# danieleschmidt/Graph-Hypernetwork-Forge

Hardware: AMD Instinct MI355X
Metric: edges/s (HyperGNN forward) (higher is better)
Workload: dtype f32; 1 GPU; synthetic uniform KG 1M nodes / 10M edges / 64 rel, hidden 128, L=3 (BASELINE config 3); nodes=1000000, edges=10000000, relations=64, hidden_dim=128, layers=3, text_dim=64, plan=cached (warm), launch=one C-ABI call per kernel, parallelism=single GPU

## Files before the change

graph-hypernetwork-forge_amd/csrc/message_bx.hip:

```cpp
#include "common.h"

#include <type_traits>

namespace ghf {

typedef float f32x4 __attribute__((ext_vector_type(4)));
typedef int i32x4 __attribute__((ext_vector_type(4)));
typedef int i32x2 __attribute__((ext_vector_type(2)));
typedef float f32x2 __attribute__((ext_vector_type(2)));
typedef _Float16 f16x8 __attribute__((ext_vector_type(8)));
typedef _Float16 f16x4 __attribute__((ext_vector_type(4)));
typedef __attribute__((address_space(3))) void* lptr_t;

template <class T>
__device__ __forceinline__ const T* bx_at(const void* base, uint32_t byte_off) {
    return (const T*)((const char*)base + byte_off);
}

__device__ __forceinline__ int lds_ld_b32(unsigned addr) {
    int v;
    asm volatile("ds_read_b32 %0, %1\n\ts_waitcnt lgkmcnt(0)" : "=&v"(v) : "v"(addr) : "memory");
    return v;
}
__device__ __forceinline__ void lds_ld_b32_x2(unsigned a0, unsigned a1, int& v0, int& v1) {
    asm volatile("ds_read_b32 %0, %2\n\tds_read_b32 %1, %3\n\ts_waitcnt lgkmcnt(0)" : "=&v"(v0), "=&v"(v1) : "v"(a0), "v"(a1) : "memory");
}
__device__ __forceinline__ void lds_ld_b32_x6(const unsigned (&a)[6], int (&v)[6]) {
    asm volatile("ds_read_b32 %0, %6\n\tds_read_b32 %1, %7\n\tds_read_b32 %2, %8\n\tds_read_b32 %3, %9\n\tds_read_b32 %4, %10\n\t"
                 "ds_read_b32 %5, %11\n\ts_waitcnt lgkmcnt(0)"
                 : "=&v"(v[0]), "=&v"(v[1]), "=&v"(v[2]), "=&v"(v[3]), "=&v"(v[4]), "=&v"(v[5])
                 : "v"(a[0]), "v"(a[1]), "v"(a[2]), "v"(a[3]), "v"(a[4]), "v"(a[5]) : "memory");
}
__device__ __forceinline__ void lds_ld_b32_x10(const unsigned (&a)[10], int (&v)[10]) {
    asm volatile("ds_read_b32 %0, %10\n\tds_read_b32 %1, %11\n\tds_read_b32 %2, %12\n\tds_read_b32 %3, %13\n\tds_read_b32 %4, %14\n\t"
                 "ds_read_b32 %5, %15\n\tds_read_b32 %6, %16\n\tds_read_b32 %7, %17\n\tds_read_b32 %8, %18\n\tds_read_b32 %9, %19\n\t"
                 "s_waitcnt lgkmcnt(0)"
                 : "=&v"(v[0]), "=&v"(v[1]), "=&v"(v[2]), "=&v"(v[3]), "=&v"(v[4]), "=&v"(v[5]), "=&v"(v[6]), "=&v"(v[7]), "=&v"(v[8]), "=&v"(v[9])
                 : "v"(a[0]), "v"(a[1]), "v"(a[2]), "v"(a[3]), "v"(a[4]), "v"(a[5]), "v"(a[6]), "v"(a[7]), "v"(a[8]), "v"(a[9]) : "memory");
}
__device__ __forceinline__ void lds_ld_b64_x2(unsigned a0, unsigned a1, f32x2& v0, f32x2& v1) {
    asm volatile("ds_read_b64 %0, %2\n\tds_read_b64 %1, %3\n\ts_waitcnt lgkmcnt(0)" : "=&v"(v0), "=&v"(v1) : "v"(a0), "v"(a1) : "memory");
}
__device__ __forceinline__ void lds_st_b32(unsigned addr, int v) { asm volatile("ds_write_b32 %0, %1" ::"v"(addr), "v"(v) : "memory"); }
__device__ __forceinline__ void lds_st_b64(unsigned addr, f32x2 v) { asm volatile("ds_write_b64 %0, %1" ::"v"(addr), "v"(v) : "memory"); }
__device__ __forceinline__ void lds_st_b128(unsigned addr, f32x4 v) { asm volatile("ds_write_b128 %0, %1" ::"v"(addr), "v"(v) : "memory"); }
#define BX_LGKM0() asm volatile("s_waitcnt lgkmcnt(0)" ::: "memory")
__device__ __forceinline__ int opaque_lane(int lane) {
    int z;
    asm volatile("v_mov_b32 %0, 0" : "=v"(z));
    return lane + z;
}

__device__ __forceinline__ int fresh_lane() {
    int z;
    asm volatile("v_mov_b32 %0, 0" : "=v"(z));
    return (int)__builtin_amdgcn_mbcnt_hi(~0u, __builtin_amdgcn_mbcnt_lo(~0u, (unsigned)z));
}

template <class T> __device__ __forceinline__ T bx_tail_ld(const T* p) { return __builtin_nontemporal_load(p); }
template <class T> __device__ __forceinline__ void bx_tail_st(T* p, T v) { __builtin_nontemporal_store(v, p); }
#define BX_IDX_WAIT "s_nop 3\n\t"
constexpr int BX_AD = 2, BX_TGB = 3;
constexpr int BX_FSPLIT = 8;

template <int D> struct BxCfg;
template <> struct BxCfg<128> {
    static constexpr int NPW = 96, CR = 76;
    static constexpr int BN = 4 * NPW;
    static constexpr int MTC = (CR + 15) / 16;
    static constexpr bool DEFER = true;
    static constexpr size_t LDS = (size_t)4 * 2 * CR * 256 + 4 * (4 * 16 * MTC + 4) * 4 + 1024 + 512 + 64;
};
template <> struct BxCfg<64> {
    static constexpr int NPW = 48, CR = 64;
    static constexpr int BN = 4 * NPW;
    static constexpr int MTC = (CR + 15) / 16;
    static constexpr bool DEFER = false;
    static constexpr size_t LDS = (size_t)4 * 2 * CR * 128 + 4 * (4 * 16 * MTC + 4) * 4 + 1024 + 512 + 64;
};

typedef float f32x32 __attribute__((ext_vector_type(32)));
typedef float f32x16 __attribute__((ext_vector_type(16)));
#define BX_PIN_128(s) "+{v[64:95]}"(s[0]), "+{v[96:127]}"(s[1]), "+{v[128:159]}"(s[2]), "+{v[160:191]}"(s[3]), "+{v[192:223]}"(s[4]), "+{v[224:255]}"(s[5])
#define BX_PIN_64(s) "+{v[64:79]}"(s[0]), "+{v[80:95]}"(s[1]), "+{v[96:111]}"(s[2])

struct BxChunk { int r; int e0; int rows; };

template <int GB_, int NV_> struct BxTailSt {
    static constexpr int GB = GB_, NV = NV_;
    f32x4 x[GB_][NV_];
    int deg[GB_];
    float gm[4 * NV_], bt[4 * NV_];
};
constexpr int BX_TCG = 8;

template <int D, int SKIP>
__global__ __launch_bounds__(512, D == 64 ? 4 : 2) void message_bx_kernel(
    const float* __restrict__ h, const void* __restrict__ h_split, int64_t N, const uint32_t* __restrict__ sorted_key,
    const int32_t* __restrict__ sorted_src, const int32_t* __restrict__ chunk_tab,
    const int32_t* __restrict__ item_tab, int64_t item0, float* __restrict__ partial,
    const int32_t* __restrict__ indeg, int R,
    const void* __restrict__ Wsplit, const float* __restrict__ bias,
    const float* __restrict__ gamma, const float* __restrict__ beta, float eps,
    int64_t row0, int64_t row_end, float* __restrict__ h_out, void* __restrict__ h_split_out, int no_tail,
    int32_t* __restrict__ range_flag, float* __restrict__ agg_out) {
    using C = BxCfg<D>;
    constexpr bool SWAP1 = SKIP == 1;
    constexpr int skip = SWAP1 ? 2 : SKIP;
    constexpr int P0_IDS = SWAP1 ? 3 : 2;
    constexpr int P0_HALF = SWAP1 ? 1 : 0;
    constexpr int BN = C::BN, MTC = C::MTC, CR = C::CR, NPW = C::NPW;
    constexpr bool DEFER = C::DEFER;
    constexpr int NWV = 8, TW = 4;
    constexpr int KS = D / 32;
    constexpr int NKS = 2 * KS;
    constexpr int NT = D / 16;
    constexpr int NTW = NT / TW;
    constexpr int NPL = 2;
    constexpr int ROWB = D * 2;
    constexpr int PLANE = CR * ROWB;
    constexpr int TILE = NPL * PLANE;
    constexpr int HROW = NPL * D * 2;
    constexpr int CRP = 16 * MTC;
    constexpr int MSTR = 4 * CRP + 4;
    constexpr int PL = D / 64;
    constexpr int TUP = D == 128 ? 32 : 16;
    constexpr int NSV = NPW * PL / TUP;
    constexpr int RPP = 1024 / ROWB;
    constexpr int LPR = 64 / RPP;
    constexpr int RBN = CR / RPP;
    constexpr int CPL = D / 16;
    constexpr int RBW = (RBN + TW - 1) / TW;
    constexpr int RPH = (CR + TW - 1) / TW;
    static_assert((NTW == 2 || NTW == 1) && CR % RPP == 0 && RPH <= 64 && NPW * TW == BN && (NPW * PL) % TUP == 0 && NPW * PL <= 192 &&
                      NPW % 2 == 0 && (BN / 2) % 4 == 0 && CR <= 128 && NSV <= 6 && (D == 128 || D == 64), "bad config");
    auto akey = [](int row) -> int { return D == 128 ? (row & 15) : ((row >> 1) & 7); };
    constexpr unsigned META_OFF = 4 * TILE,
                       DUMMY_OFF = META_OFF + 4 * MSTR * 4, ZERO_OFF = DUMMY_OFF + 1024,
                       FLAG_OFF = ZERO_OFF + 512;
    auto tile_of = [](int j) -> unsigned { return (unsigned)(j & 3) * (unsigned)TILE; };

    extern __shared__ __attribute__((aligned(16))) char smem[];
    const unsigned lds0 = (unsigned)(size_t)(lptr_t)smem;

    const int tid = threadIdx.x, lane = tid & 63;
    const int w = __builtin_amdgcn_readfirstlane(tid >> 6);
    const bool helper = w >= TW;
    const int tw = w & 3;
    const int q = lane >> 4, c16 = lane & 15;
    const i32x4 item = *(const i32x4*)(item_tab + 4 * (size_t)(item0 + blockIdx.x));
    const int64_t blk = __builtin_amdgcn_readfirstlane(item[0]);
    const int slot = __builtin_amdgcn_readfirstlane(item[3]);
    const int64_t node0 = blk * BN;
    const int nrows = (int)((row_end - node0) < BN ? (row_end - node0) : BN);
    const uint32_t seg0 = (uint32_t)(blk * R);
    const int c_begin = __builtin_amdgcn_readfirstlane(item[1]);
    const int c_end = __builtin_amdgcn_readfirstlane(item[2]);
    const int nchunks = c_end - c_begin;
    int vzero;
    asm volatile("v_mov_b32 %0, 0" : "=v"(vzero));

    auto load_desc = [&](int k) -> i32x2 {
        const int c = c_begin + (k < nchunks ? k : 0) + vzero;
        return *bx_at<i32x2>(chunk_tab, (uint32_t)c * 8u);
    };
    auto decode = [&](i32x2 d) -> BxChunk {
        const int w0 = __builtin_amdgcn_readfirstlane(d[0]), w1 = __builtin_amdgcn_readfirstlane(d[1]);
        return BxChunk{w1 >> 8, w0, w1 & 127};
    };
    auto meta_off = [&](int j) -> unsigned { return META_OFF + (unsigned)(j & 3) * (MSTR * 4); };
    const uint32_t hsc_off = (uint32_t)((uint64_t)N * HROW);

    constexpr int HN = BN / 2, HPW = NPW / 2;
    auto tail_half = [&](int half, auto gb_c) __attribute__((always_inline)) {
        const float* acc_lds = (const float*)smem;
        constexpr int CS = 64;
        const int sub = lane >> 4, c0 = 4 * (lane & 15);
        constexpr int NV = CPL / 4;
        auto node_of = [&](int v) -> int { return (v / HPW) * NPW + half * HPW + (v % HPW); };
        auto row_sum = [&](float v) -> float {
            v += dpp_take<0xB1, 0xF>(v);
            v += dpp_take<0x4E, 0xF>(v);
            v += dpp_take<0x141, 0xF>(v);
            v += dpp_take<0x140, 0xF>(v);
            return v;
        };
        auto row_max = [&](float v) -> float {
            v = fmaxf(v, dpp_take<0xB1, 0xF>(v));
            v = fmaxf(v, dpp_take<0x4E, 0xF>(v));
            v = fmaxf(v, dpp_take<0x141, 0xF>(v));
            v = fmaxf(v, dpp_take<0x140, 0xF>(v));
            return v;
        };
        constexpr int NG = HN / 4;
        if (slot >= 0) {
            float* __restrict__ ps = partial + (size_t)slot * BN * D;
            for (int g = w; g < NG; g += NWV) {
                const int v = 4 * g + sub;
                float* __restrict__ o = ps + (size_t)node_of(v) * D + c0;
#pragma unroll
                for (int i = 0; i < NV; ++i) *(f32x4*)(o + CS * i) = *(const f32x4*)(acc_lds + v * D + c0 + CS * i);
            }
            return;
        }
        float gm[CPL], bt[CPL];
#pragma unroll
        for (int c = 0; c < CPL; ++c) {
            gm[c] = no_tail ? 1.f : gamma[c0 + CS * (c >> 2) + (c & 3)];
            bt[c] = no_tail ? 0.f : beta[c0 + CS * (c >> 2) + (c & 3)];
        }
        constexpr int GB = decltype(gb_c)::value;
        for (int g0 = w; g0 < NG; g0 += NWV * GB) {
            f32x4 x[GB][NV];
            float inv[GB];
            int deg[GB];
#pragma unroll
            for (int gb = 0; gb < GB; ++gb) {
                const int g = g0 + gb * NWV;
                const int nl = node_of(4 * (g < NG ? g : NG - 1) + sub);
                const int64_t node = node0 + (nl < nrows ? nl : nrows - 1);
                deg[gb] = indeg[node];
                const float* __restrict__ hp = h + (size_t)node * D + c0;
#pragma unroll
                for (int i = 0; i < NV; ++i)
                    x[gb][i] = (no_tail && !(no_tail & GHF_FLAG_ADD_H)) ? (f32x4){0.f, 0.f, 0.f, 0.f} : bx_tail_ld((const f32x4*)(hp + CS * i));
            }
            __builtin_amdgcn_sched_barrier(0);
#pragma unroll
            for (int gb = 0; gb < GB; ++gb) inv[gb] = (no_tail & GHF_FLAG_RAW_SUM) ? 1.0f : 1.0f / (float)(deg[gb] > 1 ? deg[gb] : 1);
#pragma unroll
            for (int gb = 0; gb < GB; ++gb) {
                const int g = g0 + gb * NWV;
                const int v = 4 * (g < NG ? g : NG - 1) + sub;
                const int nl = node_of(v);
                const bool live = g < NG && nl < nrows;
                f32x4 a[NV];
#pragma unroll
                for (int i = 0; i < NV; ++i) a[i] = *(const f32x4*)(acc_lds + v * D + c0 + CS * i);
                if (agg_out && live) {
                    float* __restrict__ o = agg_out + (size_t)(node0 + nl) * D + c0;
#pragma unroll
                    for (int i = 0; i < NV; ++i) bx_tail_st((f32x4*)(o + CS * i), a[i] * inv[gb]);
                }
                float y[CPL];
                float s = 0.f;
#pragma unroll
                for (int c = 0; c < CPL; ++c) {
                    const float av = a[c >> 2][c & 3] * inv[gb];
                    y[c] = no_tail ? av + x[gb][c >> 2][c & 3] : fmaxf(av + x[gb][c >> 2][c & 3], 0.f);
                    s += y[c];
                }
                if (!no_tail) {
                    const float mean = row_sum(s) * (1.0f / D);
                    float var = 0.f;
#pragma unroll
                    for (int c = 0; c < CPL; ++c) { const float t = y[c] - mean; var += t * t; }
                    const float rstd = 1.0f / sqrtf(row_sum(var) * (1.0f / D) + eps);
#pragma unroll
                    for (int c = 0; c < CPL; ++c) y[c] = (y[c] - mean) * rstd * gm[c] + bt[c];
                }
                float up = 1.f;
                if (h_split_out) {
                    float mx = 0.f;
#pragma unroll
                    for (int c = 0; c < CPL; ++c) mx = fmaxf(mx, fabsf(y[c]));
                    const int sh = split2h_shift(row_max(mx));
                    up = pow2f(sh);
                    if ((lane & 15) == 0 && live) *(float*)((char*)h_split_out + (size_t)hsc_off + (size_t)(node0 + nl) * 4) = pow2f(-sh);
                }
                if (live) {
                    float* __restrict__ o = h_out + (size_t)(node0 + nl) * D + c0;
#pragma unroll
                    for (int i = 0; i < NV; ++i) bx_tail_st((f32x4*)(o + CS * i), (f32x4){y[4 * i], y[4 * i + 1], y[4 * i + 2], y[4 * i + 3]});
                    if (h_split_out) {
                        _Float16* __restrict__ sp = (_Float16*)h_split_out + (size_t)(node0 + nl) * (NPL * D) + c0;
                        _Float16 hi[CPL], lo[CPL];
#pragma unroll
                        for (int c = 0; c < CPL; ++c) split2h(y[c] * up, hi[c], lo[c]);
                        if constexpr (CPL == 8 && CS == 4) {
                            *(f16x8*)sp = (f16x8){hi[0], hi[1], hi[2], hi[3], hi[4], hi[5], hi[6], hi[7]};
                            *(f16x8*)(sp + D) = (f16x8){lo[0], lo[1], lo[2], lo[3], lo[4], lo[5], lo[6], lo[7]};
                        } else if constexpr (CPL == 8) {
#pragma unroll
                            for (int i = 0; i < 2; ++i) {
                                bx_tail_st((f16x4*)(sp + CS * i), (f16x4){hi[4 * i], hi[4 * i + 1], hi[4 * i + 2], hi[4 * i + 3]});
                                bx_tail_st((f16x4*)(sp + D + CS * i), (f16x4){lo[4 * i], lo[4 * i + 1], lo[4 * i + 2], lo[4 * i + 3]});
                            }
                        } else {
                            bx_tail_st((f16x4*)sp, (f16x4){hi[0], hi[1], hi[2], hi[3]});
                            bx_tail_st((f16x4*)(sp + D), (f16x4){lo[0], lo[1], lo[2], lo[3]});
                        }
                    }
                }
                if (h_split_out) {
                    int tiny = 0, nz = 0;
#pragma unroll
                    for (int c = 0; c < CPL; ++c) { tiny += range_tiny(y[c] * up); nz += y[c] != 0.f; }
                    if (__ballot(tiny != 0)) {
                        tiny = (int)row_sum((float)tiny);
                        nz = (int)row_sum((float)nz);
                        if ((lane & 15) == 0 && live) range_raise(range_flag, GHF_RANGE_ROWS, tiny, nz);
                    }
                }
            }
        }
    };

    auto tail_issue = [&](int half, auto& st, int gfirst, auto gend_c) __attribute__((always_inline)) {
        using St = typename std::remove_reference<decltype(st)>::type;
        constexpr int GB = St::GB, NV = St::NV, CS = 64;
        static_assert(NV * 4 == CPL && 4 * GB <= decltype(gend_c)::value, "one batch holds all of the wave's groups");
        if (slot >= 0) return;
        const int tl = fresh_lane(), sub = tl >> 4, c0 = 4 * (tl & 15);
        const bool no_x = no_tail && !(no_tail & GHF_FLAG_ADD_H);
        const __amdgpu_buffer_rsrc_t rsG = __builtin_amdgcn_make_buffer_rsrc((void*)gamma, 0, no_tail ? 0 : D * 4, 0x00020000);
        const __amdgpu_buffer_rsrc_t rsB = __builtin_amdgcn_make_buffer_rsrc((void*)beta, 0, no_tail ? 0 : D * 4, 0x00020000);
        const __amdgpu_buffer_rsrc_t rsX = __builtin_amdgcn_make_buffer_rsrc(
            (void*)h, 0, no_x ? 0 : (int)(uint32_t)((uint64_t)N * D * 4), 0x00020000);
#pragma unroll
        for (int c = 0; c < CPL; ++c) {
            st.gm[c] = __builtin_bit_cast(float, __builtin_amdgcn_raw_buffer_load_b32(rsG, (c0 + CS * (c >> 2) + (c & 3)) * 4, 0, 0));
            st.bt[c] = __builtin_bit_cast(float, __builtin_amdgcn_raw_buffer_load_b32(rsB, (c0 + CS * (c >> 2) + (c & 3)) * 4, 0, 0));
        }
#pragma unroll
        for (int gb = 0; gb < GB; ++gb) {
            const int v = 4 * (gfirst + 4 * gb) + sub;
            const int nl = (v / HPW) * NPW + half * HPW + (v % HPW);
            const int64_t node = node0 + (nl < nrows ? nl : nrows - 1);
            st.deg[gb] = indeg[node];
#pragma unroll
            for (int i = 0; i < NV; ++i)
                st.x[gb][i] = __builtin_bit_cast(f32x4, __builtin_amdgcn_raw_buffer_load_b128(
                    rsX, (int)(((uint32_t)node * D + c0 + CS * i) * 4u), 0, 2 ));
        }
        __builtin_amdgcn_sched_barrier(0);
    };
    auto tail_rows = [&](int half, auto& st, int gfirst, auto gend_c) __attribute__((always_inline)) {
        using St = typename std::remove_reference<decltype(st)>::type;
        constexpr int GB = St::GB, NV = St::NV, gend = decltype(gend_c)::value, CS = 64;
        __builtin_amdgcn_s_waitcnt(0x0F70);
        const float* acc_lds = (const float*)smem;
        const int tl = fresh_lane(), sub = tl >> 4, c0 = 4 * (tl & 15);
        auto node_of = [&](int v) -> int { return (v / HPW) * NPW + half * HPW + (v % HPW); };
        auto row_sum = [&](float v) -> float {
            v += dpp_take<0xB1, 0xF>(v);
            v += dpp_take<0x4E, 0xF>(v);
            v += dpp_take<0x141, 0xF>(v);
            v += dpp_take<0x140, 0xF>(v);
            return v;
        };
        auto row_max = [&](float v) -> float {
            v = fmaxf(v, dpp_take<0xB1, 0xF>(v));
            v = fmaxf(v, dpp_take<0x4E, 0xF>(v));
            v = fmaxf(v, dpp_take<0x141, 0xF>(v));
            v = fmaxf(v, dpp_take<0x140, 0xF>(v));
            return v;
        };
        if (slot >= 0) {
            float* __restrict__ ps = partial + (size_t)slot * BN * D;
            for (int g = gfirst; g < gend; g += 4) {
                const int v = 4 * g + sub;
                float* __restrict__ o = ps + (size_t)node_of(v) * D + c0;
#pragma unroll
                for (int i = 0; i < NV; ++i) *(f32x4*)(o + CS * i) = *(const f32x4*)(acc_lds + v * D + c0 + CS * i);
            }
            return;
        }
        float inv[GB];
#pragma unroll
        for (int gb = 0; gb < GB; ++gb) inv[gb] = (no_tail & GHF_FLAG_RAW_SUM) ? 1.0f : 1.0f / (float)(st.deg[gb] > 1 ? st.deg[gb] : 1);
#pragma unroll
        for (int gb = 0; gb < GB; ++gb) {
            const int v = 4 * (gfirst + 4 * gb) + sub;
            const int nl = node_of(v);
            const bool live = nl < nrows;
            f32x4 a[NV];
#pragma unroll
            for (int i = 0; i < NV; ++i) a[i] = *(const f32x4*)(acc_lds + v * D + c0 + CS * i);
            if (agg_out && live) {
                float* __restrict__ o = agg_out + (size_t)(node0 + nl) * D + c0;
#pragma unroll
                for (int i = 0; i < NV; ++i) bx_tail_st((f32x4*)(o + CS * i), a[i] * inv[gb]);
            }
            float y[CPL];
            float s = 0.f;
#pragma unroll
            for (int c = 0; c < CPL; ++c) {
                const float av = a[c >> 2][c & 3] * inv[gb];
                y[c] = no_tail ? av + st.x[gb][c >> 2][c & 3] : fmaxf(av + st.x[gb][c >> 2][c & 3], 0.f);
                s += y[c];
            }
            if (!no_tail) {
                const float mean = row_sum(s) * (1.0f / D);
                float var = 0.f;
#pragma unroll
                for (int c = 0; c < CPL; ++c) { const float t = y[c] - mean; var += t * t; }
                const float rstd = 1.0f / sqrtf(row_sum(var) * (1.0f / D) + eps);
#pragma unroll
                for (int c = 0; c < CPL; ++c) y[c] = (y[c] - mean) * rstd * st.gm[c] + st.bt[c];
            }
            float up = 1.f;
            if (h_split_out) {
                float mx = 0.f;
#pragma unroll
                for (int c = 0; c < CPL; ++c) mx = fmaxf(mx, fabsf(y[c]));
                const int sh = split2h_shift(row_max(mx));
                up = pow2f(sh);
                if ((tl & 15) == 0 && live) *(float*)((char*)h_split_out + (size_t)hsc_off + (size_t)(node0 + nl) * 4) = pow2f(-sh);
            }
            if (live) {
                float* __restrict__ o = h_out + (size_t)(node0 + nl) * D + c0;
#pragma unroll
                for (int i = 0; i < NV; ++i) bx_tail_st((f32x4*)(o + CS * i), (f32x4){y[4 * i], y[4 * i + 1], y[4 * i + 2], y[4 * i + 3]});
                if (h_split_out) {
                    _Float16* __restrict__ sp = (_Float16*)h_split_out + (size_t)(node0 + nl) * (NPL * D) + c0;
                    _Float16 hi[CPL], lo[CPL];
#pragma unroll
                    for (int c = 0; c < CPL; ++c) split2h(y[c] * up, hi[c], lo[c]);
#pragma unroll
                    for (int i = 0; i < NV; ++i) {
                        bx_tail_st((f16x4*)(sp + CS * i), (f16x4){hi[4 * i], hi[4 * i + 1], hi[4 * i + 2], hi[4 * i + 3]});
                        bx_tail_st((f16x4*)(sp + D + CS * i), (f16x4){lo[4 * i], lo[4 * i + 1], lo[4 * i + 2], lo[4 * i + 3]});
                    }
                }
            }
            if (h_split_out) {
                int tiny = 0, nz = 0;
#pragma unroll
                for (int c = 0; c < CPL; ++c) { tiny += range_tiny(y[c] * up); nz += y[c] != 0.f; }
                if (__ballot(tiny != 0)) {
                    tiny = (int)row_sum((float)tiny);
                    nz = (int)row_sum((float)nz);
                    if ((tl & 15) == 0 && live) range_raise(range_flag, GHF_RANGE_ROWS, tiny, nz);
                }
            }
        }
    };
    auto tail_barrier = [&]() __attribute__((always_inline)) {
        BX_LGKM0();
        __builtin_amdgcn_s_barrier();
        asm volatile("" ::: "memory");
    };
    constexpr int TNG = BN / 2 / 4;
    constexpr int TCG = BX_TCG, THG = TNG / 4 - TCG;
    static_assert(D != 128 || (TNG % 4 == 0 && TCG >= 1 && THG >= 1 && 9 * THG + 2 * CPL <= 96),
                  "the helpers' operands of a half fit the registers its dump freed");
    std::integral_constant<int, TNG> c_tng;
    std::integral_constant<int, 4 * TCG> c_cend;

    if (helper) {
        typename std::conditional<D == 128, f32x32, f32x16>::type sm[NSV];
#pragma unroll
        for (int k = 0; k < NSV; ++k)
#pragma unroll
            for (int i = 0; i < TUP; ++i) sm[k][i] = 0.f;
        if constexpr (D == 128) asm volatile("" : BX_PIN_128(sm)); else asm volatile("" : BX_PIN_64(sm));
        const int hw = tw;
        const __amdgpu_buffer_rsrc_t rsH = __builtin_amdgcn_make_buffer_rsrc((void*)h_split, 0, (int)hsc_off, 0x00020000);
        struct Words { int src; int key; };
        struct Scales { float u; float v; };
        auto load_words = [&](const BxChunk& c, int ln) -> Words {
            const int mrow = hw * RPH + (ln < RPH ? ln : RPH - 1);
            const int rc = mrow < c.rows ? mrow : c.rows - 1;
            const uint32_t eo = (uint32_t)(c.e0 + rc) * 4u;
            return Words{*bx_at<int>(sorted_src, eo), *bx_at<int>(sorted_key, eo)};
        };
        auto dst_of = [&](const BxChunk& c, const Words& wd) -> uint32_t {
            const uint32_t kbase = (seg0 + (uint32_t)c.r) * (uint32_t)BN;
            return (uint32_t)node0 + ((uint32_t)wd.key - kbase);
        };
        auto load_scales = [&](const BxChunk& c, const Words& wd) -> Scales {
            const uint32_t nu = (uint32_t)(wd.src & SRC_MASK), nv = dst_of(c, wd);
            return Scales{*bx_at<float>(h_split, hsc_off + nu * 4u), *bx_at<float>(h_split, hsc_off + nv * 4u)};
        };
        auto publish = [&](int j, const BxChunk& c, const Words& wd, const Scales& sc, int ln) {
            const unsigned m = lds0 + meta_off(j);
            const int mrow = hw * RPH + (ln < RPH ? ln : RPH - 1);
            if (ln < RPH && mrow < CRP) {
                lds_st_b32(m + 4 * mrow, __float_as_int(sc.u));
                lds_st_b32(m + 4 * (CRP + mrow), __float_as_int(sc.v));
                lds_st_b32(m + 4 * (2 * CRP + mrow), wd.src & SRC_MASK);
                lds_st_b32(m + 4 * (3 * CRP + mrow), (int)dst_of(c, wd));
            }
            if (hw == 0 && ln == 0) lds_st_b32(m + 4 * (4 * CRP), c.rows);
        };
        static_assert(RBW <= 6, "ids of a tile: one batched read");
        auto id_addr = [&](int j, int which , int i, int lane) -> unsigned {
            return lds0 + meta_off(j) + 4 * (which * CRP) + 4 * (RPP * (hw + TW * (i < RBW ? i : 0)) + lane / LPR);
        };
        auto dma_ids = [&](int j, int which, int lane, int (&id)[6]) {
            unsigned ia[6];
#pragma unroll
            for (int i = 0; i < 6; ++i) ia[i] = id_addr(j, which, i, lane);
            lds_ld_b32_x6(ia, id);
        };
        auto dma_issue = [&](unsigned tile_off, int rows, int lane, const int (&id)[6]) {
#pragma unroll
            for (int i_ = 0; i_ < RBW; ++i_) {
                const int i = i_;
                const int rb = hw + TW * i, row = RPP * rb + lane / LPR;
                if (RPP * rb >= rows) continue;
                const int g = (lane & (LPR - 1)) ^ akey(row);
                const int voff = row < rows ? (int)((uint32_t)id[i] * (uint32_t)HROW) + (g << 4) : (int)0xFFFFF000u;
                const unsigned dst = rb < RBN ? tile_off + (unsigned)rb * 1024u : DUMMY_OFF;
#pragma unroll
                for (int pl = 0; pl < NPL; ++pl) {
                    const unsigned d = __builtin_amdgcn_readfirstlane(dst + (rb < RBN ? pl * PLANE : 0));
                    __builtin_amdgcn_raw_ptr_buffer_load_lds(rsH, (lptr_t)(smem + d), 16, voff + pl * ROWB, 0, 0, 0);
                }
            }
        };
        auto dma_tile = [&](unsigned tile_off, int j, int which, const BxChunk& c, int lane) {
            int id[6];
            dma_ids(j, which, lane, id);
            dma_issue(tile_off, c.rows, lane, id);
        };
        struct FoldPlan { int n0, n1, ra, cnt; };
        auto fold_plan = [&](int j, int rows, int lane, int staged, bool* ready) __attribute__((always_inline)) -> FoldPlan {
            const unsigned dd = lds0 + meta_off(j) + 4 * (3 * CRP);
            const unsigned a0 = dd + 4 * lane, a1 = dd + 4 * (lane + 64 < CRP ? lane + 64 : CRP - 1);
            int d0, d1;
            if (staged > 0) {
                i32x4 f;
                asm volatile("ds_read_b32 %0, %3\n\tds_read_b32 %1, %4\n\tds_read_b128 %2, %5\n\ts_waitcnt lgkmcnt(0)"
                             : "=&v"(d0), "=&v"(d1), "=&v"(f) : "v"(a0), "v"(a1), "v"(lds0 + FLAG_OFF + 16) : "memory");
                *ready = __builtin_amdgcn_readfirstlane(min(min(f[0], f[1]), min(f[2], f[3]))) >= staged;
            } else {
                lds_ld_b32_x2(a0, a1, d0, d1);
                *ready = true;
            }
            const int base = (int)node0 + hw * NPW;
            const int n0 = d0 - base, n1 = d1 - base;
            const unsigned long long q0 = __ballot(lane < rows && (unsigned)n0 < (unsigned)NPW);
            const unsigned long long q1 = __ballot(lane + 64 < rows && (unsigned)n1 < (unsigned)NPW);
            const int cnt = __builtin_popcountll(q0) + __builtin_popcountll(q1);
            const int ra = q0 ? (int)__builtin_ctzll(q0) : 64 + (q1 ? (int)__builtin_ctzll(q1) : 0);
            return FoldPlan{n0, n1, ra, cnt};
        };
        auto fold_rows = [&](int j, const FoldPlan& fp, int lane, int g_begin, int g_end) __attribute__((always_inline)) {
            const unsigned Y = lds0 + tile_of(j - 1);
            const int ra = fp.ra, cnt = fp.cnt;
            const unsigned zrow = lds0 + ZERO_OFF + (unsigned)(PL * 4 * lane), lb = (unsigned)(PL * 4 * lane);
            typedef typename std::conditional<D == 128, f32x2, float>::type yv_t;
            constexpr int FB = 4;
            auto issue = [&](yv_t (&y)[FB], int r0) __attribute__((always_inline)) {
                unsigned a[FB];
#pragma unroll
                for (int i = 0; i < FB; ++i) {
                    const int rr = ra + r0 + i;
                    a[i] = r0 + i < cnt ? Y + (unsigned)rr * (D * 4) + (lb ^ (unsigned)(((rr >> 2) & 1) << 7)) : zrow;
                }
                if constexpr (D == 128)
                    asm volatile("ds_read_b64 %0, %4\n\tds_read_b64 %1, %5\n\tds_read_b64 %2, %6\n\tds_read_b64 %3, %7"
                                 : "=&v"(y[0]), "=&v"(y[1]), "=&v"(y[2]), "=&v"(y[3]) : "v"(a[0]), "v"(a[1]), "v"(a[2]), "v"(a[3]) : "memory");
                else
                    asm volatile("ds_read_b32 %0, %4\n\tds_read_b32 %1, %5\n\tds_read_b32 %2, %6\n\tds_read_b32 %3, %7"
                                 : "=&v"(y[0]), "=&v"(y[1]), "=&v"(y[2]), "=&v"(y[3]) : "v"(a[0]), "v"(a[1]), "v"(a[2]), "v"(a[3]) : "memory");
            };
            auto add_rows = [&](yv_t (&y)[FB], int r0, bool behind) __attribute__((always_inline)) {
                if (behind) asm volatile("s_waitcnt lgkmcnt(4)" : "+v"(y[0]), "+v"(y[1]), "+v"(y[2]), "+v"(y[3])::"memory");
                else asm volatile("s_waitcnt lgkmcnt(0)" : "+v"(y[0]), "+v"(y[1]), "+v"(y[2]), "+v"(y[3])::"memory");
                int ix[FB];
#pragma unroll
                for (int i = 0; i < FB; ++i) {
                    const int rr = ra + r0 + i;
                    const int a = __builtin_amdgcn_readlane(fp.n0, rr & 63), b = __builtin_amdgcn_readlane(fp.n1, rr & 63);
                    ix[i] = r0 + i < cnt ? PL * (rr < 64 ? a : b) : 0;
                }
                int keep;
#define BX_ROW128(i) "s_set_gpr_idx_idx %[i" #i "]\n\tv_pk_add_f32 v[64:65], %[y" #i "], v[64:65]\n\t"
#define BX_ROW64(i) "s_set_gpr_idx_idx %[i" #i "]\n\tv_add_f32 v64, %[y" #i "], v64\n\t"
#define BX_ROW_OPS [i0] "s"(ix[0]), [i1] "s"(ix[1]), [i2] "s"(ix[2]), [i3] "s"(ix[3]), [y0] "v"(y[0]), [y1] "v"(y[1]), [y2] "v"(y[2]), [y3] "v"(y[3])
                if constexpr (D == 128)
                    asm volatile("s_mov_b32 %[kp], m0\n\ts_set_gpr_idx_on %[i0], 0xa\n\t" BX_IDX_WAIT "v_pk_add_f32 v[64:65], %[y0], v[64:65]\n\t"
                                 BX_ROW128(1) BX_ROW128(2) BX_ROW128(3)
                                 "s_set_gpr_idx_off\n\t" BX_IDX_WAIT "s_mov_b32 m0, %[kp]\n\ts_nop 0"
                                 : BX_PIN_128(sm), [kp] "=&s"(keep) : BX_ROW_OPS);
                else
                    asm volatile("s_mov_b32 %[kp], m0\n\ts_set_gpr_idx_on %[i0], 0xa\n\t" BX_IDX_WAIT "v_add_f32 v64, %[y0], v64\n\t"
                                 BX_ROW64(1) BX_ROW64(2) BX_ROW64(3)
                                 "s_set_gpr_idx_off\n\t" BX_IDX_WAIT "s_mov_b32 m0, %[kp]\n\ts_nop 0"
                                 : BX_PIN_64(sm), [kp] "=&s"(keep) : BX_ROW_OPS);
#undef BX_ROW128
#undef BX_ROW64
#undef BX_ROW_OPS
            };
            for (int g = g_begin; g < cnt && g < g_end; g += 2 * FB) {
                yv_t ya[FB], yb[FB];
                issue(ya, g);
                issue(yb, g + FB);
                add_rows(ya, g, true);
                add_rows(yb, g + FB, false);
            }
        };
        auto wait_flags = [&](unsigned flags, int v) {
            for (;;) {
                i32x4 f;
                asm volatile("ds_read_b128 %0, %1\n\ts_waitcnt lgkmcnt(0)" : "=&v"(f) : "v"(flags) : "memory");
                const int lo = min(min(f[0], f[1]), min(f[2], f[3]));
                if (__builtin_amdgcn_readfirstlane(lo) >= v) break;
                __builtin_amdgcn_s_sleep(1);
            }
        };
        auto wait_flags2 = [&](unsigned fa, unsigned fb, int v) {
            for (;;) {
                i32x4 f, g;
                asm volatile("ds_read_b128 %0, %2\n\tds_read_b128 %1, %3\n\ts_waitcnt lgkmcnt(0)" : "=&v"(f), "=&v"(g) : "v"(fa), "v"(fb) : "memory");
                const int lo = min(min(min(f[0], f[1]), min(f[2], f[3])), min(min(g[0], g[1]), min(g[2], g[3])));
                if (__builtin_amdgcn_readfirstlane(lo) >= v) break;
                __builtin_amdgcn_s_sleep(1);
            }
        };

        BxChunk ch[5];
        Words wdP{0, 0}, wdN{0, 0}, wdL{0, 0};
        Scales scP{1.f, 1.f}, scN{1.f, 1.f};
        i32x2 d5{0, 0};
        if (hw == 0)
#pragma unroll
            for (int i = 0; i < 3; ++i)
                if (lane + 64 * i < 128 + 16) lds_st_b32(lds0 + ZERO_OFF + 4 * (lane + 64 * i), 0);
        int prev_rows = 1;
        if (nchunks > 0) {
            i32x2 dd[5];
#pragma unroll
            for (int j = 0; j < 5; ++j) dd[j] = load_desc(j);
#pragma unroll
            for (int j = 0; j < 5; ++j) ch[j] = decode(dd[j]);
            Words wd[4];
            Scales sc[3];
#pragma unroll
            for (int j = 0; j < 4; ++j) wd[j] = load_words(ch[j], lane);
#pragma unroll
            for (int j = 0; j < 3; ++j) sc[j] = load_scales(ch[j], wd[j]);
#pragma unroll
            for (int j = 0; j < 2; ++j) publish(j, ch[j], wd[j], sc[j], lane);
            wdP = wd[2];
            scP = sc[2];
            wdN = wd[3];
        }
        BX_LGKM0();
        __builtin_amdgcn_s_barrier();
        if (nchunks > 0) {
            if (!(skip & 1)) dma_tile(tile_of(0), 0, P0_IDS, ch[0], lane);
            if (!(skip & 2)) dma_tile(tile_of(-1), 0, 3, ch[0], lane);
            asm volatile("s_waitcnt vmcnt(0)" ::: "memory");
        }
        int sid[6] = {0, 0, 0, 0, 0, 0};
        if (nchunks > 0 && !(skip & 1)) dma_ids(1, P0_IDS, lane, sid);
        for (int k = 0; k < nchunks; ++k) {
            __builtin_amdgcn_s_barrier();
            const int l0 = opaque_lane(lane);
            if (k > 0) {
                wdP = wdN;
                scP = scN;
                wdN = wdL;
#pragma unroll
                for (int j = 0; j < 4; ++j) ch[j] = ch[j + 1];
                ch[4] = decode(d5);
                asm volatile("" : "+v"(wdP.src), "+v"(wdP.key), "+v"(scP.u), "+v"(scP.v), "+v"(wdN.src), "+v"(wdN.key));
            }
            publish(k + 2, ch[2], wdP, scP, l0);
            if (!(skip & 1)) dma_issue(tile_of(k + 1), ch[1].rows, l0, sid);
            BX_LGKM0();
            if (lane == 0) lds_st_b32(lds0 + FLAG_OFF + 4 * hw, k + 1);
            FoldPlan fp{0, 0, 0, 0};
            if (k > 0) {
                bool staged;
                fp = fold_plan(k - 1, prev_rows, l0, DEFER ? k : 0, &staged);
                if (DEFER && !staged) wait_flags(lds0 + FLAG_OFF + 16, k);
                fold_rows(k - 1, fp, l0, 0, BX_FSPLIT);
            }
            int did[6];
            if (!(skip & 2)) {
                dma_ids(k + 1, 3, opaque_lane(lane), did);
                wait_flags2(lds0 + FLAG_OFF, lds0 + FLAG_OFF + 32, k + 1);
            } else {
                wait_flags(lds0 + FLAG_OFF, k + 1);
            }
            const int l1 = opaque_lane(lane);
            scN = load_scales(ch[3], wdN);
            wdL = load_words(ch[4], l1);
            d5 = load_desc(k + 5);
            if (!(skip & 2)) dma_issue(tile_of(k), ch[1].rows, l1, did);
            fold_rows(k - 1, fp, l1, BX_FSPLIT, CR + 8);
            prev_rows = ch[0].rows;
            if (!(skip & 1)) dma_ids(k + 2, P0_IDS, l1, sid);
            asm volatile("s_waitcnt vmcnt(0)" ::: "memory");
            BX_LGKM0();
        }
        __builtin_amdgcn_s_barrier();
        if (nchunks > 0) {
            const int le = opaque_lane(lane);
            bool staged;
            fold_rows(nchunks - 1, fold_plan(nchunks - 1, prev_rows, le, 0, &staged), le, 0, CR + 8);
        }
        asm volatile("s_waitcnt vmcnt(0)" ::: "memory");
        BX_LGKM0();
        if constexpr (D == 128) asm volatile("" : BX_PIN_128(sm)); else asm volatile("" : BX_PIN_64(sm));
        auto dump_half = [&](auto half_c) __attribute__((always_inline)) {
            constexpr int H = decltype(half_c)::value;
            float* __restrict__ o = (float*)smem + (size_t)(hw * HPW) * D + (D == 128 ? 32 * (lane >> 4) + (lane & 15) : lane);
#pragma unroll
            for (int i = 0; i < HPW; ++i)
#pragma unroll
                for (int e = 0; e < PL; ++e) {
                    const int reg = PL * (H * HPW + i) + e;
                    o[i * D + 16 * e] = sm[reg / TUP][reg % TUP];
                }
        };
        __syncthreads();
        dump_half(std::integral_constant<int, 0>{});
        if constexpr (D == 128) {
            const int gf = 4 * TCG + hw;
            BxTailSt<THG, CPL / 4> st;
            tail_issue(0, st, gf, c_tng);
            tail_barrier();
            tail_rows(0, st, gf, c_tng);
            tail_issue(1, st, gf, c_tng);
            tail_barrier();
            dump_half(std::integral_constant<int, 1>{});
            tail_barrier();
            tail_rows(1, st, gf, c_tng);
        } else {
            BX_LGKM0();
            __syncthreads();
            tail_half(0, std::integral_constant<int, 1>{});
            __syncthreads();
            dump_half(std::integral_constant<int, 1>{});
            BX_LGKM0();
            __syncthreads();
            tail_half(1, std::integral_constant<int, BX_TGB>{});
        }
    } else {
        const uint32_t wsc_off = (uint32_t)((uint64_t)R * 2 * D * D * (NPL * 2));
        const __amdgpu_buffer_rsrc_t rsW = __builtin_amdgcn_make_buffer_rsrc((void*)Wsplit, 0, (int)wsc_off, 0x00020000);
        auto b_soff = [&](int r, int ph, int t) -> int {
            return __builtin_amdgcn_readfirstlane((((r * NT + tw * NTW + t) * NKS + ph * KS) * NPL) * 1024);
        };
        const int lane16 = lane * 16;
        i32x4 b[KS][NTW][NPL];
        auto load_b_step = [&](int r, int ph, int j) {
#pragma unroll
            for (int t = 0; t < NTW; ++t)
#pragma unroll
                for (int pl = 0; pl < NPL; ++pl)
                    b[j][t][pl] = __builtin_amdgcn_raw_buffer_load_b128(rsW, lane16 + pl * 1024, b_soff(r, ph, t) + j * (NPL * 1024), 0);
        };
        f32x4 acc[MTC][NTW];
        const int arow = c16 * ROWB;
        constexpr int AD = BX_AD;
        static_assert(AD <= MTC - 2, "the prefetched positions are row tiles 0 .. AD-1 of the first k-step in every instance");
        i32x4 apre[AD][NPL];
        auto lda_from = [&](const char* Abuf, int j, int m, i32x4 (&dst)[NPL]) __attribute__((always_inline)) {
            const char* src = Abuf + arow + (((4 * j + q) ^ akey(c16)) << 4) + m * 16 * ROWB;
#pragma unroll
            for (int pl = 0; pl < NPL; ++pl) dst[pl] = *(const i32x4*)(src + pl * PLANE);
        };
        auto prefetch_a = [&](const char* Abuf) __attribute__((always_inline)) {
#pragma unroll
            for (int p = 0; p < AD; ++p) lda_from(Abuf, 0, p, apre[p]);
        };
        auto compute_stage = [&](auto mt_c, auto pre_c, int ph, bool first, const char* Abuf, const int* meta, float wscale, int r_next, int ph_next,
                                 const float (&bias_v)[NTW], auto&& after_k) __attribute__((always_inline)) {
            constexpr int MT = decltype(mt_c)::value;
            constexpr bool PRE = decltype(pre_c)::value;
            f32x4 part[MTC][NTW];
#pragma unroll
            for (int m = 0; m < MT; ++m)
#pragma unroll
                for (int t = 0; t < NTW; ++t) part[m][t] = (f32x4){0.f, 0.f, 0.f, 0.f};
            f32x4 sc[MTC];
            i32x4 a[AD + 1][NPL];
            auto lda = [&](int j, int m, i32x4 (&dst)[NPL]) { lda_from(Abuf, j, m, dst); };
#pragma unroll
            for (int p = 0; p < AD && p < KS * MT; ++p) {
                if constexpr (PRE) {
#pragma unroll
                    for (int pl = 0; pl < NPL; ++pl) a[p][pl] = apre[p][pl];
                } else {
                    lda(p / MT, p % MT, a[p]);
                }
            }
#pragma unroll
            for (int j = 0; j < KS; ++j) {
                if (j == KS - 1) {
#pragma unroll
                    for (int m = 0; m < MT; ++m) sc[m] = *(const f32x4*)(meta + ph * CRP + m * 16 + 4 * q);
                }
#pragma unroll
                for (int m = 0; m < MT; ++m) {
                    const int p = j * MT + m, cur = p % (AD + 1);
                    if (p + AD < KS * MT) lda((p + AD) / MT, (p + AD) % MT, a[(p + AD) % (AD + 1)]);
#pragma unroll
                    for (int t = 0; t < NTW; ++t) {
                        auto fma = [&](int pa, int pb) {
                            part[m][t] = __builtin_amdgcn_mfma_f32_16x16x32_f16(__builtin_bit_cast(f16x8, a[cur][pa]),
                                                                                __builtin_bit_cast(f16x8, b[j][t][pb]),
                                                                                part[m][t], 0, 0, 0);
                        };
                        fma(1, 0); fma(0, 1);
                        fma(0, 0);
                    }
                }
                __builtin_amdgcn_sched_barrier(0);
                load_b_step(r_next, ph_next, j);
                __builtin_amdgcn_sched_barrier(0);
            }
            after_k();
#pragma unroll
            for (int m = 0; m < MT; ++m) {
#pragma unroll
                for (int s = 0; s < 4; ++s) {
                    const float f = sc[m][s] * wscale;
#pragma unroll
                    for (int t = 0; t < NTW; ++t) acc[m][t][s] = fmaf(part[m][t][s], f, first ? bias_v[t] : acc[m][t][s]);
                }
            }
#pragma unroll
            for (int m = MT; m < MTC; ++m)
#pragma unroll
                for (int t = 0; t < NTW; ++t) acc[m][t] = (f32x4){0.f, 0.f, 0.f, 0.f};
        };
        auto stage_for = [&](int mt, auto pre_c, int ph, bool first, const char* Abuf, const int* meta, float wscale, int r_next, int ph_next,
                             const float (&bias_v)[NTW], auto&& after_k) __attribute__((always_inline)) {
            static_assert(MTC >= 3, "three compute_stage instances");
            if (mt >= MTC) compute_stage(std::integral_constant<int, MTC>{}, pre_c, ph, first, Abuf, meta, wscale, r_next, ph_next, bias_v, after_k);
            else if (mt == MTC - 1) compute_stage(std::integral_constant<int, MTC - 1>{}, pre_c, ph, first, Abuf, meta, wscale, r_next, ph_next, bias_v, after_k);
            else compute_stage(std::integral_constant<int, MTC - 2>{}, pre_c, ph, first, Abuf, meta, wscale, r_next, ph_next, bias_v, after_k);
        };
        const unsigned yoff = (unsigned)(4 * q) * (D * 4) + (unsigned)((((NTW == 2 ? 32 * tw + 2 * c16 : 16 * tw + c16)) ^ ((q & 1) << 5)) * 4);
        auto write_rows = [&](int mt, unsigned ytile) __attribute__((always_inline)) {
            const unsigned ybase = lds0 + ytile + yoff;
#pragma unroll
            for (int m = 0; m < MTC; ++m) {
                if (m >= mt) continue;
                if (16 * m + 16 > CR && 16 * m + 4 * q >= CR) continue;
#pragma unroll
                for (int s = 0; s < 4; ++s) {
                    if constexpr (NTW == 2)
                        asm volatile("ds_write_b64 %0, %1 offset:%2" ::"v"(ybase), "v"((f32x2){acc[m][0][s], acc[m][NTW - 1][s]}),
                                     "n"((16 * m + s) * (D * 4)) : "memory");
                    else
                        asm volatile("ds_write_b32 %0, %1 offset:%2" ::"v"(ybase), "v"(acc[m][0][s]), "n"((16 * m + s) * (D * 4)) : "memory");
                }
            }
        };

        const int ph_first = (skip & 1) ? 1 : P0_HALF;
        BxChunk ch{0, 0, 1};
        i32x2 dn{0, 0};
        float bias_v[NTW] = {}, bias_n[NTW] = {}, wscale = 1.f, wscale_n = 1.f;
        auto load_rel_words = [&](int r, float& ws, float (&bv)[NTW]) {
            ws = *bx_at<float>(Wsplit, wsc_off + (uint32_t)(r + vzero) * 4u);
#pragma unroll
            for (int t = 0; t < NTW; ++t) bv[t] = *bx_at<float>(bias, (uint32_t)(r * D + (tw * NTW + t) * 16 + c16) * 4u);
        };
        int mt_prev = 0;
        if (nchunks > 0) {
            ch = decode(load_desc(0));
            dn = load_desc(1);
            load_rel_words(ch.r, wscale, bias_v);
#pragma unroll
            for (int j = 0; j < KS; ++j) load_b_step(ch.r, ph_first, j);
        }
        __syncthreads();
        for (int k = 0; k < nchunks; ++k) {
            const int mt = (ch.rows + 15) >> 4;
            const int* meta = (const int*)(smem + meta_off(k));
            __syncthreads();
            if (DEFER && k > 0) {
                write_rows(mt_prev, tile_of(k - 2));
                BX_LGKM0();
                if (lane == 0) lds_st_b32(lds0 + FLAG_OFF + 16 + 4 * tw, k);
            }
            const BxChunk nx = decode(dn);
            constexpr bool PRE1 = false;
            static_assert(!PRE1, "the hook has no flag words of its own any more: wait_landed spins on words that mean something else (a hung CU)");
            auto wait_landed = [&]() __attribute__((always_inline)) {
                for (;;) {
                    i32x4 f;
                    asm volatile("ds_read_b128 %0, %1\n\ts_waitcnt lgkmcnt(0)" : "=&v"(f) : "v"(lds0 + FLAG_OFF) : "memory");
                    const int lo = min(min(f[0], f[1]), min(f[2], f[3]));
                    if (__builtin_amdgcn_readfirstlane(lo) >= k + 1) break;
                    __builtin_amdgcn_s_sleep(1);
                }
            };
            auto next_pre = [&]() __attribute__((always_inline)) {
                if (PRE1) {
                    wait_landed();
                    prefetch_a(smem + tile_of(k - 1));
                }
                if (!(skip & 2) && lane == 0) lds_st_b32(lds0 + FLAG_OFF + 32 + 4 * tw, k + 1);
            };
            auto no_after = []() {};
            if (!(skip & 1))
                stage_for(mt, std::false_type{}, P0_HALF, true, smem + tile_of(k), meta, wscale, (skip & 2) ? nx.r : ch.r, (skip & 2) ? P0_HALF : 1, bias_v, next_pre);
            dn = load_desc(k + 2);
            load_rel_words(nx.r, wscale_n, bias_n);
            if (skip & 1) {
#pragma unroll
                for (int m = 0; m < MTC; ++m)
#pragma unroll
                    for (int t = 0; t < NTW; ++t) acc[m][t] = (f32x4){bias_v[t], bias_v[t], bias_v[t], bias_v[t]};
            }
            if (!(skip & 2)) stage_for(mt, std::false_type{}, 1, false, smem + tile_of(k - 1), meta, wscale, nx.r, ph_first, bias_v, no_after);
            const bool stage_now = !DEFER || k + 1 == nchunks;
            if (stage_now) {
                const unsigned fw = DEFER ? FLAG_OFF + 48 : FLAG_OFF + 16;
                const int fv = DEFER ? 1 : k + 1;
                if (lane == 0) lds_st_b32(lds0 + fw + 4 * tw, fv);
                for (;;) {
                    i32x4 f;
                    asm volatile("ds_read_b128 %0, %1\n\ts_waitcnt lgkmcnt(0)" : "=&v"(f) : "v"(lds0 + fw) : "memory");
                    const int lo = min(min(f[0], f[1]), min(f[2], f[3]));
                    if (__builtin_amdgcn_readfirstlane(lo) >= fv) break;
                    __builtin_amdgcn_s_sleep(1);
                }
                write_rows(mt, tile_of(k - 1));
            }
            mt_prev = mt;
            ch = nx;
            wscale = wscale_n;
#pragma unroll
            for (int t = 0; t < NTW; ++t) bias_v[t] = bias_n[t];
            BX_LGKM0();
        }
        __syncthreads();
        if constexpr (D == 128) {
            BxTailSt<TCG, CPL / 4> st;
            tail_issue(0, st, tw, c_cend);
            tail_barrier();
            tail_barrier();
            tail_rows(0, st, tw, c_cend);
            tail_issue(1, st, tw, c_cend);
            tail_barrier();
            tail_barrier();
            tail_rows(1, st, tw, c_cend);
        } else {
            for (int half = 0; half < 2; ++half) {
                __syncthreads();
                __syncthreads();
                tail_half(half, std::integral_constant<int, BX_TGB>{});
            }
        }
    }
}

template <int D>
static int launch_bx_for(const MsgArgs& a, hipStream_t stream) {
    using C = BxCfg<D>;
    constexpr size_t lds = C::LDS;
    static_assert(lds <= 160 * 1024, "LDS budget");
    static_assert((size_t)(C::BN / 2) * D * 4 <= (size_t)3 * 2 * C::CR * (D * 2), "the tail's dump of half a block must fit three whole tiles of the ring");
    GHF_REQUIRE(a.block_nodes == C::BN, "message(bx): plan block_nodes=%d, kernel for d=%d needs %d", a.block_nodes, D, C::BN);
    GHF_REQUIRE(a.wlayout == GHF_WLAYOUT_SPLIT2H, "message(bx): weights must be in SPLIT2H layout");
    GHF_REQUIRE(a.chunk_tab && a.item_tab && a.blk_item_off, "message(bx): the plan's chunk / item tables are missing");
    GHF_REQUIRE(a.h_split, "message(bx): h_split is missing (ghf_split_rows)");
    const int64_t row_end = a.row0 + a.rows;
    GHF_REQUIRE(row_end == a.N || row_end % C::BN == 0, "message(bx): row range must end on a block boundary or at N");
    if (a.rows <= 0) return GHF_OK;
    GHF_REQUIRE((uint64_t)a.N * (D * 4 + 4) <= 0xFFFFF000ull && (uint64_t)a.E * 4 < (1ull << 32) &&
                    (uint64_t)a.R * (2 * D * D * 4 + 4) < (1ull << 32),
                "message(bx): 32-bit byte offsets need N*(4d+4) <= 4 GiB - 4 KiB, E*4 and R*(8d*d+4) below 4 GiB");
    GHF_REQUIRE(a.n_items >= cdiv(a.rows, C::BN), "message(bx): n_items=%lld is fewer than the blocks of the row range", (long long)a.n_items);
    GHF_REQUIRE(a.n_items == cdiv(a.rows, C::BN) || a.partial, "message(bx): split blocks need the `partial` scratch");
    const int skip = ((a.flags & GHF_FLAG_ZERO_SRC) ? 1 : 0) | ((a.flags & GHF_FLAG_ZERO_DST) ? 2 : 0);
    const size_t lds_dyn = lds;
    auto go = [&](auto skip_c) {
        constexpr int S = decltype(skip_c)::value;
        GHF_SET_MAX_LDS((message_bx_kernel<D, S>), lds_dyn);
        message_bx_kernel<D, S><<<(unsigned)a.n_items, 512, lds_dyn, stream>>>(a.h, a.h_split, a.N, a.sorted_key, a.sorted_src, a.chunk_tab, a.item_tab,
                                                                          a.item0, a.partial, a.indeg, a.R, a.W_msg, a.bias, a.ln_gamma,
                                                                          a.ln_beta, a.ln_eps, a.row0, row_end, a.h_out, a.h_split_out,
                                                                          a.flags & (GHF_FLAG_NO_TAIL | GHF_FLAG_RAW_SUM | GHF_FLAG_ADD_H), range_flag_ptr(), a.agg_out);
        return GHF_OK;
    };
    if (skip == 1) go(std::integral_constant<int, 1>{});
    else if (skip == 2) go(std::integral_constant<int, 2>{});
    else go(std::integral_constant<int, 0>{});
    GHF_LAUNCH_CHECK();
    if (a.n_items > cdiv(a.rows, C::BN)) return launch_combine_split(a, stream);
    return GHF_OK;
}

__global__ __launch_bounds__(256) void split2h_rows_kernel(const float* __restrict__ h, int64_t N, int64_t row0, int64_t rows,
                                                           int d, char* __restrict__ out, int32_t* __restrict__ range_flag) {
    const int lane = threadIdx.x & 63;
    const int64_t i = (int64_t)blockIdx.x * 4 + (threadIdx.x >> 6);
    if (i >= rows) return;
    const int64_t row = row0 + i;
    const float* __restrict__ src = h + row * d;
    float mx = 0.f;
    for (int k = lane; k < d; k += 64) mx = fmaxf(mx, fabsf(src[k]));
    const int sh = split2h_shift(wave_absmax(mx));
    const float up = pow2f(sh);
    _Float16* __restrict__ dst = (_Float16*)(out + row * (4 * (int64_t)d));
    int tiny = 0, nz = 0;
    for (int k = lane; k < d; k += 64) {
        _Float16 hi, lo;
        const float xs = src[k] * up;
        split2h(xs, hi, lo);
        dst[k] = hi;
        dst[d + k] = lo;
        tiny += __popcll(__ballot(range_tiny(xs)));
        nz += __popcll(__ballot(xs != 0.f));
    }
    if (lane == 0) {
        *(float*)(out + N * (4 * (int64_t)d) + row * 4) = pow2f(-sh);
        range_raise(range_flag, GHF_RANGE_ROWS, tiny, nz);
    }
}

int launch_split2h_rows(const float* h, int64_t N, int d, int64_t row0, int64_t rows, void* h_split, hipStream_t stream) {
    if (rows <= 0) return GHF_OK;
    GHF_REQUIRE(cdiv(rows, 4) < (1ll << 31), "split_rows: too many rows per launch");
    split2h_rows_kernel<<<(unsigned)cdiv(rows, 4), 256, 0, stream>>>(h, N, row0, rows, d, (char*)h_split, range_flag_ptr());
    GHF_LAUNCH_CHECK();
    return GHF_OK;
}

bool message_bx_config(int d, int* block_nodes, int* chunk_rows, int* split_chunks) {
    if (d != 128 && d != 64) return false;
    *block_nodes = d == 128 ? BxCfg<128>::BN : BxCfg<64>::BN;
    *chunk_rows = d == 128 ? BxCfg<128>::CR : BxCfg<64>::CR;
    *split_chunks = 128;
    return true;
}

bool message_bx_owns(int d, int block_nodes) {
    return (d == 128 && block_nodes == BxCfg<128>::BN) || (d == 64 && block_nodes == BxCfg<64>::BN);
}

int launch_message_bx(const MsgArgs& a, hipStream_t stream) {
    if (a.d == 128) return launch_bx_for<128>(a, stream);
    if (a.d == 64) return launch_bx_for<64>(a, stream);
    return set_err(GHF_EUNSUPPORTED, "message(bx): no kernel for d=%d", a.d);
}

}
```

Measured before the change: 1.099 billion edges/s.

## Deepen metadata ring to five slots and fold flag polling into row fold

The per-chunk metadata ring in LDS grows from four to five slots, so publishing of chunk k+3 metadata moves to the end of the iteration, after the DMA and fold work, instead of happening at the top with a lane-0 flag store. The helper-wave flag check is piggybacked on the first fold batch as an extra ds_read_b128, which removes the separate wait_flags2 spin loop in the common case. The next chunk's ID reads are merged into one asm block with the vmcnt wait. The intent is to cut synchronisation stalls and barrier-bound latency per chunk, at the cost of more LDS per workgroup, which could limit occupancy (a static_assert guards the hidden-64 case).

```diff
diff --git a/graph-hypernetwork-forge_amd/csrc/message_bx.hip b/graph-hypernetwork-forge_amd/csrc/message_bx.hip
--- a/graph-hypernetwork-forge_amd/csrc/message_bx.hip
+++ b/graph-hypernetwork-forge_amd/csrc/message_bx.hip
@@ -69,15 +69,16 @@
     static constexpr int BN = 4 * NPW;
     static constexpr int MTC = (CR + 15) / 16;
     static constexpr bool DEFER = true;
-    static constexpr size_t LDS = (size_t)4 * 2 * CR * 256 + 4 * (4 * 16 * MTC + 4) * 4 + 1024 + 512 + 64;
+    static constexpr size_t LDS = (size_t)4 * 2 * CR * 256 + 5 * (4 * 16 * MTC + 4) * 4 + 1024 + 512 + 64;
 };
 template <> struct BxCfg<64> {
     static constexpr int NPW = 48, CR = 64;
     static constexpr int BN = 4 * NPW;
     static constexpr int MTC = (CR + 15) / 16;
     static constexpr bool DEFER = false;
-    static constexpr size_t LDS = (size_t)4 * 2 * CR * 128 + 4 * (4 * 16 * MTC + 4) * 4 + 1024 + 512 + 64;
+    static constexpr size_t LDS = (size_t)4 * 2 * CR * 128 + 5 * (4 * 16 * MTC + 4) * 4 + 1024 + 512 + 64;
 };
+static_assert(2 * BxCfg<64>::LDS <= 160 * 1024, "hidden 64: two workgroups per CU share the LDS");
 
 typedef float f32x32 __attribute__((ext_vector_type(32)));
 typedef float f32x16 __attribute__((ext_vector_type(16)));
@@ -136,7 +137,7 @@
                       NPW % 2 == 0 && (BN / 2) % 4 == 0 && CR <= 128 && NSV <= 6 && (D == 128 || D == 64), "bad config");
     auto akey = [](int row) -> int { return D == 128 ? (row & 15) : ((row >> 1) & 7); };
     constexpr unsigned META_OFF = 4 * TILE,
-                       DUMMY_OFF = META_OFF + 4 * MSTR * 4, ZERO_OFF = DUMMY_OFF + 1024,
+                       DUMMY_OFF = META_OFF + 5 * MSTR * 4, ZERO_OFF = DUMMY_OFF + 1024,
                        FLAG_OFF = ZERO_OFF + 512;
     auto tile_of = [](int j) -> unsigned { return (unsigned)(j & 3) * (unsigned)TILE; };
 
@@ -168,7 +169,7 @@
         const int w0 = __builtin_amdgcn_readfirstlane(d[0]), w1 = __builtin_amdgcn_readfirstlane(d[1]);
         return BxChunk{w1 >> 8, w0, w1 & 127};
     };
-    auto meta_off = [&](int j) -> unsigned { return META_OFF + (unsigned)(j & 3) * (MSTR * 4); };
+    auto meta_off = [&](int j) -> unsigned { return META_OFF + ((unsigned)j % 5u) * (MSTR * 4); };
     const uint32_t hsc_off = (uint32_t)((uint64_t)N * HROW);
 
     constexpr int HN = BN / 2, HPW = NPW / 2;
@@ -537,7 +538,7 @@
             const int ra = q0 ? (int)__builtin_ctzll(q0) : 64 + (q1 ? (int)__builtin_ctzll(q1) : 0);
             return FoldPlan{n0, n1, ra, cnt};
         };
-        auto fold_rows = [&](int j, const FoldPlan& fp, int lane, int g_begin, int g_end) __attribute__((always_inline)) {
+        auto fold_rows = [&](int j, const FoldPlan& fp, int lane, int g_begin, int g_end, i32x4* pf) __attribute__((always_inline)) {
             const unsigned Y = lds0 + tile_of(j - 1);
             const int ra = fp.ra, cnt = fp.cnt;
             const unsigned zrow = lds0 + ZERO_OFF + (unsigned)(PL * 4 * lane), lb = (unsigned)(PL * 4 * lane);
@@ -557,8 +558,9 @@
                     asm volatile("ds_read_b32 %0, %4\n\tds_read_b32 %1, %5\n\tds_read_b32 %2, %6\n\tds_read_b32 %3, %7"
                                  : "=&v"(y[0]), "=&v"(y[1]), "=&v"(y[2]), "=&v"(y[3]) : "v"(a[0]), "v"(a[1]), "v"(a[2]), "v"(a[3]) : "memory");
             };
-            auto add_rows = [&](yv_t (&y)[FB], int r0, bool behind) __attribute__((always_inline)) {
-                if (behind) asm volatile("s_waitcnt lgkmcnt(4)" : "+v"(y[0]), "+v"(y[1]), "+v"(y[2]), "+v"(y[3])::"memory");
+            auto add_rows = [&](yv_t (&y)[FB], int r0, bool behind, i32x4* landed) __attribute__((always_inline)) {
+                if (landed) asm volatile("s_waitcnt lgkmcnt(4)" : "+v"(y[0]), "+v"(y[1]), "+v"(y[2]), "+v"(y[3]), "+v"(*landed)::"memory");
+                else if (behind) asm volatile("s_waitcnt lgkmcnt(4)" : "+v"(y[0]), "+v"(y[1]), "+v"(y[2]), "+v"(y[3])::"memory");
                 else asm volatile("s_waitcnt lgkmcnt(0)" : "+v"(y[0]), "+v"(y[1]), "+v"(y[2]), "+v"(y[3])::"memory");
                 int ix[FB];
 #pragma unroll
@@ -587,10 +589,11 @@
             };
             for (int g = g_begin; g < cnt && g < g_end; g += 2 * FB) {
                 yv_t ya[FB], yb[FB];
+                if (pf) asm volatile("ds_read_b128 %0, %1" : "=&v"(*pf) : "v"(lds0 + FLAG_OFF + 32) : "memory");
                 issue(ya, g);
                 issue(yb, g + FB);
-                add_rows(ya, g, true);
-                add_rows(yb, g + FB, false);
+                add_rows(ya, g, true, pf);
+                add_rows(yb, g + FB, false, nullptr);
             }
         };
         auto wait_flags = [&](unsigned flags, int v) {
@@ -602,19 +605,10 @@
                 __builtin_amdgcn_s_sleep(1);
             }
         };
-        auto wait_flags2 = [&](unsigned fa, unsigned fb, int v) {
-            for (;;) {
-                i32x4 f, g;
-                asm volatile("ds_read_b128 %0, %2\n\tds_read_b128 %1, %3\n\ts_waitcnt lgkmcnt(0)" : "=&v"(f), "=&v"(g) : "v"(fa), "v"(fb) : "memory");
-                const int lo = min(min(min(f[0], f[1]), min(f[2], f[3])), min(min(g[0], g[1]), min(g[2], g[3])));
-                if (__builtin_amdgcn_readfirstlane(lo) >= v) break;
-                __builtin_amdgcn_s_sleep(1);
-            }
-        };
 
         BxChunk ch[5];
-        Words wdP{0, 0}, wdN{0, 0}, wdL{0, 0};
-        Scales scP{1.f, 1.f}, scN{1.f, 1.f};
+        Words wdN{0, 0}, wdL{0, 0};
+        Scales scN{1.f, 1.f};
         i32x2 d5{0, 0};
         if (hw == 0)
 #pragma unroll
@@ -634,9 +628,7 @@
 #pragma unroll
             for (int j = 0; j < 3; ++j) sc[j] = load_scales(ch[j], wd[j]);
 #pragma unroll
-            for (int j = 0; j < 2; ++j) publish(j, ch[j], wd[j], sc[j], lane);
-            wdP = wd[2];
-            scP = sc[2];
+            for (int j = 0; j < 3; ++j) publish(j, ch[j], wd[j], sc[j], lane);
             wdN = wd[3];
         }
         BX_LGKM0();
@@ -652,48 +644,54 @@
             __builtin_amdgcn_s_barrier();
             const int l0 = opaque_lane(lane);
             if (k > 0) {
-                wdP = wdN;
-                scP = scN;
                 wdN = wdL;
 #pragma unroll
                 for (int j = 0; j < 4; ++j) ch[j] = ch[j + 1];
                 ch[4] = decode(d5);
-                asm volatile("" : "+v"(wdP.src), "+v"(wdP.key), "+v"(scP.u), "+v"(scP.v), "+v"(wdN.src), "+v"(wdN.key));
-            }
-            publish(k + 2, ch[2], wdP, scP, l0);
+                asm volatile("" : "+v"(wdN.src), "+v"(wdN.key));
+            }
             if (!(skip & 1)) dma_issue(tile_of(k + 1), ch[1].rows, l0, sid);
-            BX_LGKM0();
-            if (lane == 0) lds_st_b32(lds0 + FLAG_OFF + 4 * hw, k + 1);
             FoldPlan fp{0, 0, 0, 0};
+            bool p0_read = false;
             if (k > 0) {
                 bool staged;
                 fp = fold_plan(k - 1, prev_rows, l0, DEFER ? k : 0, &staged);
                 if (DEFER && !staged) wait_flags(lds0 + FLAG_OFF + 16, k);
-                fold_rows(k - 1, fp, l0, 0, BX_FSPLIT);
+                i32x4 pf = {0, 0, 0, 0};
+                fold_rows(k - 1, fp, l0, 0, BX_FSPLIT, (skip & 2) ? nullptr : &pf);
+                if (!(skip & 2) && fp.cnt > 0) p0_read = __builtin_amdgcn_readfirstlane(min(min(pf[0], pf[1]), min(pf[2], pf[3]))) >= k + 1;
             }
             int did[6];
             if (!(skip & 2)) {
                 dma_ids(k + 1, 3, opaque_lane(lane), did);
-                wait_flags2(lds0 + FLAG_OFF, lds0 + FLAG_OFF + 32, k + 1);
-            } else {
-                wait_flags(lds0 + FLAG_OFF, k + 1);
+                if (!p0_read) wait_flags(lds0 + FLAG_OFF + 32, k + 1);
             }
             const int l1 = opaque_lane(lane);
             scN = load_scales(ch[3], wdN);
             wdL = load_words(ch[4], l1);
             d5 = load_desc(k + 5);
             if (!(skip & 2)) dma_issue(tile_of(k), ch[1].rows, l1, did);
-            fold_rows(k - 1, fp, l1, BX_FSPLIT, CR + 8);
+            fold_rows(k - 1, fp, l1, BX_FSPLIT, CR + 8, nullptr);
             prev_rows = ch[0].rows;
-            if (!(skip & 1)) dma_ids(k + 2, P0_IDS, l1, sid);
-            asm volatile("s_waitcnt vmcnt(0)" ::: "memory");
+            if (!(skip & 1)) {
+                unsigned ia[6];
+#pragma unroll
+                for (int i = 0; i < 6; ++i) ia[i] = id_addr(k + 2, P0_IDS, i, l1);
+                asm volatile("ds_read_b32 %0, %6\n\tds_read_b32 %1, %7\n\tds_read_b32 %2, %8\n\tds_read_b32 %3, %9\n\tds_read_b32 %4, %10\n\t"
+                             "ds_read_b32 %5, %11\n\ts_waitcnt vmcnt(0)\n\ts_waitcnt lgkmcnt(0)"
+                             : "=&v"(sid[0]), "=&v"(sid[1]), "=&v"(sid[2]), "=&v"(sid[3]), "=&v"(sid[4]), "=&v"(sid[5])
+                             : "v"(ia[0]), "v"(ia[1]), "v"(ia[2]), "v"(ia[3]), "v"(ia[4]), "v"(ia[5]) : "memory");
+            } else {
+                asm volatile("s_waitcnt vmcnt(0)" ::: "memory");
+            }
+            publish(k + 3, ch[3], wdN, scN, l1);
             BX_LGKM0();
         }
         __builtin_amdgcn_s_barrier();
         if (nchunks > 0) {
             const int le = opaque_lane(lane);
             bool staged;
-            fold_rows(nchunks - 1, fold_plan(nchunks - 1, prev_rows, le, 0, &staged), le, 0, CR + 8);
+            fold_rows(nchunks - 1, fold_plan(nchunks - 1, prev_rows, le, 0, &staged), le, 0, CR + 8, nullptr);
         }
         asm volatile("s_waitcnt vmcnt(0)" ::: "memory");
         BX_LGKM0();
```

Result: no change. 1.096 billion edges/s (-0.3%).
